# JiehongLin/SAM-6D

Hardware: AMD Instinct MI355X
Metric: RGB-D frames/sec (SAM-6D per-frame hot path: SAM ViT-H encoder + ISM scoring + PEM) (higher is better)
Workload: dtype bf16 (SAM ViT-H: 87 % of the step) + f16 (PEM ViT-B feature extractor) + f32 (ISM scoring, PEM point transformer and pose solvers); 1 GPU; LM-O single object: 32 frames/step/GPU, 640x480 RGB-D -> 1024^2 SAM input, P=128 proposals x 42 templates (scored in groups of 8 frames), 1 instance/frame, 2048 pts (PEM batch 32); sam_frames_per_launch_group=16, pem_vit_dtype=fp16 (set by bench.py; the library default is fp32)

## Files before the change

### include/sam6d_hip.h

```cpp
#ifndef SAM6D_HIP_H
#define SAM6D_HIP_H

#include <stdint.h>

#ifdef __cplusplus
extern "C" {
#endif

#define S6D_OK 0
#define S6D_EINVAL (-1)
#define S6D_ELAUNCH (-2)
#define S6D_EUNSUPPORTED (-3)

#define S6D_ABI_VERSION 136
int s6d_version(void);
int s6d_set_persistent_grid_limit(int max_workgroups);
int s6d_set_gemm_wave_tile(int columns);
int s6d_set_gemm_mfma_shape(int rows);
int s6d_set_gemm_small_tile(int enable);
const char *s6d_strerror(int code);
const char *s6d_last_hip_error(void);


int s6d_fps_f32(const float *xyz, int B, int N, int M, float *tmp, int32_t *idx, void *stream);

int s6d_gather_points_f32(const float *points, const int32_t *idx, int B, int C, int N, int M,
                          float *out, void *stream);

int s6d_ball_query_f32(const float *new_xyz, const float *xyz, int B, int N, int M, float radius,
                       int nsample, int32_t *idx, void *stream);

int s6d_group_points_f32(const float *points, const int32_t *idx, int B, int C, int N, int M, int S,
                         float *out, void *stream);

int s6d_gather_rows_f32(const float *src, const int32_t *idx, int B, int N, int C, int M, float *out,
                        void *stream);

int s6d_segment_seq_sum_f32(const float *x, const int64_t *start, const int64_t *count, int P, int C, float *out,
                            void *stream);

int s6d_pem_sample_indices_f32(const float *keys, long key_stride, const int64_t *count, int P, int n_sample,
                               int64_t *idx, int32_t *overflow, void *stream);

int s6d_pem_mask_boxes_u8(const unsigned char *mask, const float *depth, int P, int H, int W, long min_points,
                          unsigned char *m, int64_t *cnt, unsigned char *ok, int64_t *box, void *stream);

int s6d_pem_compact_cloud_f32(const unsigned char *m, const float *depth, const int64_t *box, const unsigned char *ok, int P,
                              int H, int W, float fx, float fy, float cx, float cy, long cap, int32_t *choose, float *cloud,
                              int64_t *n, void *stream);
int s6d_pem_radius_filter_f32(const float *center, const double *limit, int P, long cap, int32_t *choose, float *cloud,
                              int64_t *n, void *stream);

int s6d_pem_crops_f32(const unsigned char *image, const unsigned char *m, const int64_t *kept, const int64_t *box, int M,
                      int H, int W, int S, int use_mask, const float *mean3_host, const float *std3_host, float *out,
                      void *stream);


int s6d_template_boxes_u8(const unsigned char *mask, int T, int H, int W, int64_t *cnt, int64_t *box, int64_t *tight,
                          void *stream);

int s6d_template_points_f32(const unsigned char *mask, const float *xyz_mm, const int64_t *box, int T, int H, int W, long cap,
                            int32_t *choose, float *pts, int64_t *n, void *stream);

int s6d_template_pem_crops_f32(const unsigned char *images, const unsigned char *mask, const int64_t *box, int T, int H, int W,
                               int S, int use_mask, const float *mean3_host, const float *std3_host, float *out, void *stream);

int s6d_template_ism_crops_f32(const unsigned char *images, const unsigned char *mask, const void *params, int T, int H, int W,
                               int S, int normalize, const float *mean3_host, const float *std3_host, float *out_rgb,
                               float *out_mask, void *stream);


int s6d_raster_views_f32(const float *vertices, const int32_t *faces, const unsigned char *colors, const float *poses, int V, int F,
                         int T, int H, int W, float fx, float fy, float cx, float cy, float znear, float ambient, float diffuse,
                         void *workspace, unsigned char *rgb, unsigned char *mask, float *xyz, float *depth, int32_t *face,
                         int32_t *skipped, void *stream);
long s6d_raster_workspace_bytes(int T, int F, int H, int W);

int s6d_texture_pyramid_u8(const unsigned char *image, int Ht, int Wt, void *pyramid, void *stream);
long s6d_texture_pyramid_bytes(int Ht, int Wt);

int s6d_raster_views_tex_f32(const float *vertices, const int32_t *faces, const float *uv, const void *pyramid, const float *poses,
                             int V, int F, int T, int H, int W, int Ht, int Wt, float fx, float fy, float cx, float cy, float znear,
                             float ambient, float diffuse, void *workspace, unsigned char *rgb, unsigned char *mask, float *xyz,
                             float *depth, int32_t *face, int32_t *level, int32_t *skipped, void *stream);

int s6d_raster_depth_f32(const float *vertices, const int32_t *faces, const float *poses, const float *cams, int V, int F, int T,
                         int H, int W, float znear, void *workspace, float *depth, int32_t *skipped, void *stream);
long s6d_raster_depth_workspace_bytes(int T, int F, int H, int W);


int s6d_pose_err_mssd_mspd_f32(const float *vertices, const float *est, const float *gts, const float *cams, int V, int N, int S,
                               float *mssd, float *mspd, void *stream);

int s6d_vsd_counts_f32(const float *depth_est, const float *depth_gt, const float *depth_test, const int32_t *test_index,
                       const float *cams, const float *scale, int N, int M, int H, int W, float delta, const float *taus_host,
                       int NT, int32_t *uni, int32_t *inter, int32_t *ge, void *stream);

int s6d_gt_visibility_f32(const float *canvas, const float *depth_test, const int32_t *test_index, const float *cams, int N, int M,
                          int H, int W, int mx, int my, float delta, uint8_t *mask, uint8_t *mask_visib, int32_t *counts,
                          int32_t *extents, void *stream);

int s6d_model_diameter_f32(const float *vertices, int V, float *diameter, void *stream);
// ... 282 lines not shown
```

### sam6d_amd/csrc/s6d_attn_common.h

```cpp
#pragma once
#include "s6d_bf16.h"

#ifndef S6D_ATTN_F16
#define S6D_ATTN_F16 0
#endif
#if S6D_ATTN_F16
#define S6D_ATTN_NS s6d_h
#define S6D_ATTN_MFMA16(a, b, c) __builtin_amdgcn_mfma_f32_16x16x32_f16(a, b, c, 0, 0, 0)
#define S6D_ATTN_ONE 0x3C00
#else
#define S6D_ATTN_NS s6d
#define S6D_ATTN_MFMA16(a, b, c) __builtin_amdgcn_mfma_f32_16x16x32_bf16(a, b, c, 0, 0, 0)
#define S6D_ATTN_ONE 0x3F80
#endif

namespace S6D_ATTN_NS {
using namespace s6d;

#if S6D_ATTN_F16
typedef f16x8 bf16x8;
__device__ __forceinline__ u16 f2bf(float f) {
  union { _Float16 b; u16 u; } x;
  x.b = (_Float16)f;
  return x.u;
// ... 149 lines not shown
  union PB { bf16x8 v; u16 h[8]; };
  PB pb[NS][2];
  union VA { bf16x8 v; s16x4 q[2]; };
  if (PRIO) __builtin_amdgcn_s_setprio(0);
  if (kAbl & 4) {
#pragma unroll
    for (int n = 0; n < NS; ++n)
#pragma unroll
      for (int sub = 0; sub < 4; ++sub)
#pragma unroll
        for (int r = 0; r < 4; ++r) pb[n][sub >> 1].h[(sub & 1) * 4 + r] = f2bf(s[n][sub][r]);
  } else {
    constexpr float kDefer = 6.0f;
    float mx[NS];
    bool grow[NS], any_grow = false;
#pragma unroll
    for (int n = 0; n < NS; ++n) {
      float v = s[n][0][0];
#pragma unroll
      for (int sub = 0; sub < SUBS; ++sub)
#pragma unroll
        for (int r = 0; r < 4; ++r) v = fmaxf(v, s[n][sub][r]);
      v = fmaxf(v, __shfl_xor(v, 16));
      v = fmaxf(v, __shfl_xor(v, 32));
      if (MODE == 1) v += thv[n];
      mx[n] = v;
      grow[n] = __any(v - st.m_run[n] > kDefer);
      any_grow |= grow[n];
    }
    S6D_TICK(tk, 3);
    if (any_grow) {
#pragma unroll
      for (int n = 0; n < NS; ++n)
        if (grow[n]) {
          const float m_new = fmaxf(st.m_run[n], mx[n]);
          const float alpha = fast_exp2(st.m_run[n] - m_new);
          st.lacc[n] *= alpha;
#pragma unroll
          for (int dt = 0; dt < C::DT; ++dt) st.oacc[n][dt] *= alpha;
          st.m_run[n] = m_new;
        }
    }
#pragma unroll
    for (int n = 0; n < NS; ++n) {
      const float m_sub = (MODE == 1) ? st.m_run[n] - thv[n] : st.m_run[n];
#pragma unroll
      for (int sub = 0; sub < 4; ++sub)
#pragma unroll
        for (int r = 0; r < 4; ++r)
          pb[n][sub >> 1].h[(sub & 1) * 4 + r] = sub < SUBS ? f2bf(fast_exp2(s[n][sub][r] - m_sub)) : (u16)0;
    }
  }
  if (kAbl & 8) {
#pragma unroll
    for (int n = 0; n < NS; ++n) st.lacc[n][0] += (float)pb[n][0].h[0] + (float)pb[n][1].h[7];
    return;
  }
  union { bf16x8 v; u16 h[8]; } ones;
#pragma unroll
  for (int i = 0; i < 8; ++i) ones.h[i] = S6D_ATTN_ONE;
  S6D_TICK(tk, 4);
  if (PRIO) __builtin_amdgcn_s_setprio(1);
#pragma unroll
  for (int j = 0; j < (SUBS + 1) / 2; ++j) {
    const u16 *vrow = Vl + (32 * j + g * 4 + (c >> 2)) * C::VROW + (c & 3) * 4;
#pragma unroll
    for (int n = 0; n < NS; ++n) st.lacc[n] = S6D_ATTN_MFMA16(ones.v, pb[n][j].v, st.lacc[n]);
#pragma unroll
    for (int dt = 0; dt < C::DT; ++dt) {
      VA va;
      va.q[0] = __builtin_amdgcn_ds_read_tr16_b64_v4i16((S6D_LDS(s16x4) *)(vrow + dt * 16));
      va.q[1] = __builtin_amdgcn_ds_read_tr16_b64_v4i16((S6D_LDS(s16x4) *)(vrow + 16 * C::VROW + dt * 16));
#pragma unroll
      for (int n = 0; n < NS; ++n)
        st.oacc[n][dt] = S6D_ATTN_MFMA16(va.v, pb[n][j].v, st.oacc[n][dt]);
    }
  }
  if (PRIO) __builtin_amdgcn_s_setprio(0);
}

constexpr float kNoMaxSumLimit = 1.2676506e30f;
constexpr float kNoMaxFinite = 3.0e38f;

template <int HD, int NS, bool KSWZ>
__device__ __forceinline__ void process_tile_nomax(const AttnParams &p, const u16 *Kl, const u16 *Vl, StripState<HD, NS> &st,
                                                   const f32x4 (&cbias)[NS][4], const float (&nb)[NS], int lane) {
  using C = Cfg<HD>;
  const int g = lane >> 4, c = lane & 15;
  const int gk = KSWZ ? (g ^ kswz(c)) : g;
  union PB { bf16x8 v; u16 h[8]; };
  PB pb[NS][2];
#pragma unroll
  for (int sub = 0; sub < 4; ++sub) {
    f32x4 acc[NS];
#pragma unroll
    for (int n = 0; n < NS; ++n) acc[n] = cbias[n][sub];
#pragma unroll
    for (int ks = 0; ks < C::KS; ++ks) {
      const bf16x8 a = *reinterpret_cast<const bf16x8 *>(Kl + (sub * 16 + c) * C::KROW + ks * 32 + gk * 8);
#pragma unroll
      for (int n = 0; n < NS; ++n) acc[n] = S6D_ATTN_MFMA16(a, st.qf[n][ks], acc[n]);
    }
#pragma unroll
    for (int n = 0; n < NS; ++n)
#pragma unroll
      for (int r = 0; r < 4; ++r)
        pb[n][sub >> 1].h[(sub & 1) * 4 + r] = f2bf(fast_exp2(__builtin_fmaf(acc[n][r], p.scale_log2, nb[n])));
  }
  union { bf16x8 v; u16 h[8]; } ones;
#pragma unroll
  for (int i = 0; i < 8; ++i) ones.h[i] = S6D_ATTN_ONE;
  union VA { bf16x8 v; s16x4 q[2]; };
#pragma unroll
  for (int j = 0; j < 2; ++j) {
    const u16 *vrow = Vl + (32 * j + g * 4 + (c >> 2)) * C::VROW + (c & 3) * 4;
#pragma unroll
    for (int n = 0; n < NS; ++n) st.lacc[n] = S6D_ATTN_MFMA16(ones.v, pb[n][j].v, st.lacc[n]);
#pragma unroll
    for (int dt = 0; dt < C::DT; ++dt) {
      VA va;
      va.q[0] = __builtin_amdgcn_ds_read_tr16_b64_v4i16((S6D_LDS(s16x4) *)(vrow + dt * 16));
      va.q[1] = __builtin_amdgcn_ds_read_tr16_b64_v4i16((S6D_LDS(s16x4) *)(vrow + 16 * C::VROW + dt * 16));
#pragma unroll
      for (int n = 0; n < NS; ++n) st.oacc[n][dt] = S6D_ATTN_MFMA16(va.v, pb[n][j].v, st.oacc[n][dt]);
    }
  }
}

template <int HD, int THREADS>
struct Stager {
  using C = Cfg<HD>;
  static constexpr int NK = (64 * C::KPARTS + THREADS - 1) / THREADS;
  static constexpr int NV = (64 * C::VPARTS + THREADS - 1) / THREADS;
  uint4 k[NK], v[NV];

  __device__ __forceinline__ void load(const AttnParams &p, int b, int wy, int wx, int head, int key0, int tid) {
#pragma unroll
    for (int n = 0; n < NK; ++n) {
      const int i = min(tid + n * THREADS, 64 * C::KPARTS - 1);
      const int key = i / C::KPARTS, part = i - key * C::KPARTS;
      size_t tok;
      const bool valid = token_offset(p, b, wy, wx, key0 + key, tok);
      k[n] = load_chunk<HD>(p, 1, head, valid, tok, part * 8);
    }
#pragma unroll
    for (int n = 0; n < NV; ++n) {
      const int i = min(tid + n * THREADS, 64 * C::VPARTS - 1);
      const int key = i / C::VPARTS, part = i - key * C::VPARTS;
      size_t tok;
      const bool valid = token_offset(p, b, wy, wx, key0 + key, tok);
      v[n] = load_chunk<HD>(p, 2, head, valid, tok, part * 8);
    }
  }
  __device__ __forceinline__ void store(u16 *Kl, u16 *Vl, int tid, int klim = 64, int vlim = 64) const {
#pragma unroll
    for (int n = 0; n < NK; ++n) {
      const int i = tid + n * THREADS;
      const int key = i / C::KPARTS, part = i - key * C::KPARTS;
      if (i < 64 * C::KPARTS && key < klim) *reinterpret_cast<uint4 *>(Kl + key * C::KROW + part * 8) = k[n];
    }
#pragma unroll
    for (int n = 0; n < NV; ++n) {
      const int i = tid + n * THREADS;
      const int key = i / C::VPARTS, part = i - key * C::VPARTS;
      if (i < 64 * C::VPARTS && key < vlim) *reinterpret_cast<uint4 *>(Vl + key * C::VROW + part * 8) = v[n];
    }
  }
};

template <int HD, int THREADS>
struct StagerLinear {
  using C = Cfg<HD>;
  static constexpr int NK = (64 * C::KPARTS + THREADS - 1) / THREADS;
  static constexpr int NV = (64 * C::VPARTS + THREADS - 1) / THREADS;
  uint4 k[NK], v[NV];
  const u16 *kp[NK], *vp[NV];
  int ko[NK], vo[NV];
  bool kz[NK];
  static_assert(Cfg<HD>::KROW - Cfg<HD>::HDP == 8, "K rows end in a 16-byte pad");

  __device__ __forceinline__ void init(const AttnParams &p, int b, int head, int tid) {
#pragma unroll
    for (int n = 0; n < NK; ++n) {
      const int i = tid + n * THREADS, ic = min(i, 64 * C::KPARTS - 1);
      const int key = ic / C::KPARTS, part = ic - key * C::KPARTS;
      kz[n] = part * 8 >= HD;
      kp[n] = qkv_at(p, (size_t)b * p.T + key, 1, head) + (kz[n] ? HD - 8 : part * 8);
      ko[n] = i < 64 * C::KPARTS ? key * C::KROW + (part ^ kswz(key)) * 8 : (tid & 63) * C::KROW + C::HDP;
    }
#pragma unroll
    for (int n = 0; n < NV; ++n) {
      const int i = tid + n * THREADS, ic = min(i, 64 * C::VPARTS - 1);
      const int key = ic / C::VPARTS, part = ic - key * C::VPARTS;
      vp[n] = qkv_at(p, (size_t)b * p.T + key, 2, head) + part * 8;
      vo[n] = i < 64 * C::VPARTS ? 64 * C::KROW + key * C::VROW + part * 8 : (tid & 63) * C::KROW + C::HDP;
    }
  }
  __device__ __forceinline__ void load(size_t tile_stride_elems, int t) {
#pragma unroll
    for (int n = 0; n < NK; ++n) k[n] = *reinterpret_cast<const uint4 *>(kp[n] + tile_stride_elems * t);
#pragma unroll
    for (int n = 0; n < NV; ++n) v[n] = *reinterpret_cast<const uint4 *>(vp[n] + tile_stride_elems * t);
  }
  __device__ __forceinline__ void store(u16 *Kl) const {
#pragma unroll
    for (int n = 0; n < NK; ++n) *reinterpret_cast<uint4 *>(Kl + ko[n]) = kz[n] ? make_uint4(0, 0, 0, 0) : k[n];
#pragma unroll
    for (int n = 0; n < NV; ++n) *reinterpret_cast<uint4 *>(Kl + vo[n]) = v[n];
  }
// ... 90 lines not shown
```

### sam6d_amd/csrc/s6d_attn_global.h

```cpp
#pragma once
#include "s6d_attn_common.h"

namespace S6D_ATTN_NS {

constexpr bool kGlbPrio = true;

template <int HD, int WAVES, int MODE>
__global__ __launch_bounds__(WAVES * 64) void attn_global_kernel(AttnParams p) {
  using C = Cfg<HD>;
  constexpr int NS = 2;
  static_assert(MODE == 0 || MODE == 2, "attn_global_kernel: table bias (0) or no bias (2); the 64 x 64 grid is attn_global64_kernel's");
  S6D_DYN_LDS(smem);
  constexpr int KBYTES = 64 * C::KROW * 2, VBYTES = 64 * C::VROW * 2;
  auto Kbuf = [&](int r) { return reinterpret_cast<u16 *>(smem + r * (KBYTES + VBYTES)); };
  auto Vbuf = [&](int r) { return reinterpret_cast<u16 *>(smem + r * (KBYTES + VBYTES) + KBYTES); };
  float *tabs = reinterpret_cast<float *>(smem + 2 * (KBYTES + VBYTES));
  const int tid = threadIdx.x, wave = tid >> 6, lane = tid & 63;
  const int c = lane & 15;

  const int nqt = (p.T + WAVES * 16 * NS - 1) / (WAVES * 16 * NS);
  int id = blockIdx.x;
  const int nbh = p.B * p.nh;
  int qt, bh;
  if ((nbh & 7) == 0) {
    const int xcd = id & 7, loc = id >> 3;
    qt = loc % nqt;
    bh = (loc / nqt) * 8 + xcd;
  } else {
    qt = id % nqt;
    bh = id / nqt;
  }
  const int head = bh % p.nh, b = bh / p.nh;
  StripState<HD, NS> st;
  int q0[NS];
#pragma unroll
  for (int n = 0; n < NS; ++n) {
    q0[n] = ((qt * WAVES + wave) * NS + n) * 16;
    load_q<HD>(p, b, 0, 0, head, q0[n], st.qf[n], lane);
    const int qi = min(q0[n] + c, p.T - 1);
    st.qy[n] = div_S(p, qi);
    st.qx[n] = qi - st.qy[n] * p.S;
    st.m_run[n] = -1e30f;
    st.lacc[n] = f32x4{0.f, 0.f, 0.f, 0.f};
#pragma unroll
    for (int i = 0; i < 16; ++i) st.twr[n][i] = 0.f;
#pragma unroll
    for (int dt = 0; dt < C::DT; ++dt) st.oacc[n][dt] = f32x4{0.f, 0.f, 0.f, 0.f};
    st.th[n] = nullptr;
    st.tw[n] = nullptr;
  }
  if (MODE == 0) {
#pragma unroll
    for (int n = 0; n < NS; ++n) {
      float *th = tabs + (size_t)(wave * NS + n) * 2 * 16 * p.LT, *tw = th + 16 * p.LT;
      for (int jt = 0; jt < p.LT / 16; ++jt) {
        build_table<HD, 1>(p.rel_h, jt * 16, 1, st.qf[n], th + jt * 16, p.LT, lane);
        build_table<HD, 1>(p.rel_w, jt * 16, 1, st.qf[n], tw + jt * 16, p.LT, lane);
      }
      st.th[n] = th;
      st.tw[n] = tw;
    }
  }
  const int ntile = p.T / 64;
  StagerLinear<HD, WAVES * 64> sg;
  sg.init(p, b, head, tid);
  const size_t tstride = (size_t)64 * (size_t)p.tok_stride;
  sg.load(tstride, 0);
  __syncthreads();
  sg.store(Kbuf(0));
  __syncthreads();
  auto tile = [&](int t) {
    const float thv[NS] = {0.f, 0.f};
    if (!(kAbl & 2)) process_tile<HD, MODE, NS, true, kGlbPrio>(p, Kbuf(t & 1), Vbuf(t & 1), t * 64, st, thv, lane);
  };
  for (int t = 0; t + 1 < ntile; ++t) {
    if (!(kAbl & 1)) sg.load(tstride, t + 1);
    tile(t);
    if (!(kAbl & 32)) sg.store(Kbuf((t & 1) ^ 1));
    __syncthreads();
  }
  tile(ntile - 1);
#pragma unroll
  for (int n = 0; n < NS; ++n) store_strip<HD>(p, b, 0, 0, head, q0[n], st.lacc[n][0], st.oacc[n], lane);
}

constexpr int G64_THLD = 65;
#ifndef S6D_G64_SLOTS
#define S6D_G64_SLOTS 3
#endif
#ifndef S6D_G64_WAVES
#define S6D_G64_WAVES 8
#endif
#ifndef S6D_G64_NOMAX
#define S6D_G64_NOMAX 1
#endif

template <int HD, int WAVES_, int SLOTS_>
struct G64 {
  using C = Cfg<HD>;
  static constexpr int WAVES = WAVES_, NS = 2, SLOTS = SLOTS_;
  static constexpr int KCH = C::KROW / 8, VCH = C::VROW / 8;
  static constexpr int NPIECE = KCH + VCH;
  static constexpr int PW = (NPIECE + WAVES - 1) / WAVES;
  static constexpr int SLOT = NPIECE * 1024;
  static constexpr int RING = SLOTS * SLOT;
  static constexpr int TABS = WAVES * NS * 16 * G64_THLD * 4;
  static constexpr int LDS = RING + TABS + 16;
  static_assert(NPIECE > WAVES * (PW - 1) && PW >= 2, "every wave has a real piece to repeat");
  static_assert(RING >= WAVES * 16 * 80 * 4, "the prologue's per-wave scratch aliases the ring");
  static_assert(PW * (SLOTS - 2) <= 15 || SLOTS == 2, "vmcnt immediates used below");
};

template <int PW>
__device__ __forceinline__ void g64_wait_tiles(int n) {
  switch (PW * n) {
#define S6D_G64_CASE(k) case k: S6D_VMCNT(k); break;
    S6D_G64_CASE(0) S6D_G64_CASE(3) S6D_G64_CASE(5) S6D_G64_CASE(6) S6D_G64_CASE(9) S6D_G64_CASE(10) S6D_G64_CASE(12)
#undef S6D_G64_CASE
    default: S6D_VMCNT(15); break;
  }
}

template <int HD, int WAVES, int SLOTS>
__global__ __launch_bounds__(WAVES * 64) void attn_global64_kernel(AttnParams p) {
  using C = Cfg<HD>;
  using G = G64<HD, WAVES, SLOTS>;
  constexpr int NS = G::NS, PW = G::PW;
  S6D_DYN_LDS(smem);
  float *tabs = reinterpret_cast<float *>(smem + G::RING);
  const int tid = threadIdx.x, wave = __builtin_amdgcn_readfirstlane(tid >> 6), lane = tid & 63;
  const int g = lane >> 4, c = lane & 15;
  const int nqt = p.T / (WAVES * 16 * NS);
  const int nbh = p.B * p.nh;
  int id = blockIdx.x, qt, bh;
  if ((nbh & 7) == 0) {
    const int xcd = id & 7, loc = id >> 3;
    qt = loc % nqt;
    bh = (loc / nqt) * 8 + xcd;
  } else {
    qt = id % nqt;
    bh = id / nqt;
  }
  const int head = bh % p.nh, b = bh / p.nh;
  StripState<HD, NS> st;
  int q0[NS];
  float *thm[NS];
#pragma unroll
  for (int n = 0; n < NS; ++n) {
    q0[n] = ((qt * WAVES + wave) * NS + n) * 16;
    load_q<HD>(p, b, 0, 0, head, q0[n], st.qf[n], lane);
    st.qy[n] = q0[n] >> 6;
    st.qx[n] = (q0[n] & 63) + c;
    st.m_run[n] = -1e30f;
    st.lacc[n] = f32x4{0.f, 0.f, 0.f, 0.f};
#pragma unroll
    for (int dt = 0; dt < C::DT; ++dt) st.oacc[n][dt] = f32x4{0.f, 0.f, 0.f, 0.f};
    st.th[n] = nullptr;
    st.tw[n] = nullptr;
    float *th = tabs + (size_t)(wave * NS + n) * 16 * G64_THLD;
    float *Gs = reinterpret_cast<float *>(smem) + (size_t)wave * 16 * 80;
    const int q0y = q0[n] >> 6, q0x = q0[n] & 63;
    build_table<HD, 4>(p.rel_h, q0y + 63, -1, st.qf[n], th, G64_THLD, lane);
    build_table<HD, 5>(p.rel_w, q0x, 1, st.qf[n], Gs, 80, lane);
    S6D_WAVE_RENDEZVOUS();
#pragma unroll
    for (int sub = 0; sub < 4; ++sub)
#pragma unroll
      for (int r = 0; r < 4; ++r) st.twr[n][sub * 4 + r] = Gs[c * 80 + (c + 63 - (sub * 16 + g * 4 + r))];
    S6D_WAVE_RENDEZVOUS();
    thm[n] = th;
  }
  const u16 *src[PW];
  long inc[PW];
  int dsto[PW];
  const long tstride = 64L * p.tok_stride;
#pragma unroll
  for (int i = 0; i < PW; ++i) {
    const int q = wave + WAVES * i < G::NPIECE ? wave + WAVES * i : wave + WAVES * (i - 1);
    const bool isk = q < G::KCH;
    const int piece = isk ? q : q - G::KCH, rowch = isk ? G::KCH : G::VCH;
    const int j = piece * 64 + lane;
    const int row = j / rowch, pp = j - row * rowch;
    const int part = isk ? (pp < C::KPARTS ? pp ^ kswz(row) : C::KPARTS) : pp;
    const bool data = part * 8 < HD;
    src[i] = data ? qkv_at(p, (size_t)b * p.T + row, isk ? 1 : 2, head) + part * 8 : reinterpret_cast<const u16 *>(&g_attn_zero16);
    inc[i] = data ? tstride : 0;
    dsto[i] = q * 1024;
  }
  auto issue = [&](int slot) __attribute__((always_inline)) {
#pragma unroll
    for (int i = 0; i < PW; ++i) {
      S6D_LDS(char) *dst = (S6D_LDS(char) *)smem + slot * G::SLOT + dsto[i];
      lds_dma16_m0(src[i], dst);
      src[i] += inc[i];
    }
  };
  const int ntile = p.T / 64;
  constexpr int D = SLOTS - 1;
  static_assert(D >= 1 && D <= 6, "ring depth");
  f32x4 cbias[NS][4];
  {
    const float inv = 1.0f / p.scale_log2;
#pragma unroll
    for (int n = 0; n < NS; ++n)
#pragma unroll
      for (int sub = 0; sub < 4; ++sub)
#pragma unroll
        for (int r = 0; r < 4; ++r) cbias[n][sub][r] = st.twr[n][sub * 4 + r] * inv;
  }
  int *redo = reinterpret_cast<int *>(smem + G::RING + G::TABS);
  const u16 *src0[PW];
#pragma unroll
  for (int i = 0; i < PW; ++i) src0[i] = src[i];
  long long tk[6] = {0, 0, 0, 0, 0, 0}, tsum[5] = {0, 0, 0, 0, 0};
  int slot = 0;
  auto tile_head = [&](int t, float (&thv)[NS]) __attribute__((always_inline)) -> const u16 * {
    S6D_TICK(tk, 0);
    g64_wait_tiles<PW>(min(D - 1, ntile - 1 - t));
    S6D_LGKM0();
    __builtin_amdgcn_s_barrier();
    S6D_TICK(tk, 1);
    if (t + D < ntile && !(kAbl & 1)) issue(slot >= 1 ? slot - 1 : SLOTS - 1);
#pragma unroll
    for (int n = 0; n < NS; ++n) thv[n] = thm[n][c * G64_THLD + t];
    S6D_TICK(tk, 2);
    const u16 *Kl = reinterpret_cast<const u16 *>(smem + slot * G::SLOT);
    slot = slot == SLOTS - 1 ? 0 : slot + 1;
    return Kl;
  };
  auto prime = [&]() __attribute__((always_inline)) {
    __syncthreads();
    if (tid == 0) *redo = 0;
#pragma unroll
    for (int d = 0; d < D; ++d) issue(d);
    slot = 0;
  };
  bool done = false;
  if (S6D_G64_NOMAX && !S6D_G64_TIMING) {
    prime();
    {
      float thv[NS];
      const u16 *Kl = tile_head(0, thv);
      process_tile<HD, 1, NS, true, kGlbPrio>(p, Kl, Kl + 64 * C::KROW, 0, st, thv, lane, tk);
    }
    for (int t = 1; t < ntile; ++t) {
      float thv[NS], nb[NS];
      const u16 *Kl = tile_head(t, thv);
#pragma unroll
      for (int n = 0; n < NS; ++n) nb[n] = thv[n] - st.m_run[n];
      process_tile_nomax<HD, NS, true>(p, Kl, Kl + 64 * C::KROW, st, cbias, nb, lane);
    }
    bool bad = false;
#pragma unroll
    for (int n = 0; n < NS; ++n) {
      bad |= !(st.lacc[n][0] < kNoMaxSumLimit);
#pragma unroll
      for (int dt = 0; dt < C::DT; ++dt)
#pragma unroll
        for (int r = 0; r < 4; ++r) bad |= !(fabsf(st.oacc[n][dt][r]) < kNoMaxFinite);
    }
    if (__any(bad) && lane == 0) *redo = 1;
    __syncthreads();
    done = *redo == 0;
    if (!done) {
#pragma unroll
      for (int n = 0; n < NS; ++n) {
        st.m_run[n] = -1e30f;
        st.lacc[n] = f32x4{0.f, 0.f, 0.f, 0.f};
#pragma unroll
        for (int dt = 0; dt < C::DT; ++dt) st.oacc[n][dt] = f32x4{0.f, 0.f, 0.f, 0.f};
      }
#pragma unroll
      for (int i = 0; i < PW; ++i) src[i] = src0[i];
    }
  }
  if (!done) {
    prime();
    for (int t = 0; t < ntile; ++t) {
      float thv[NS];
      const u16 *Kl = tile_head(t, thv);
      if (!(kAbl & 2)) process_tile<HD, 1, NS, true, kGlbPrio>(p, Kl, Kl + 64 * C::KROW, t * 64, st, thv, lane, tk);
      S6D_TICK(tk, 5);
      if (S6D_G64_TIMING)
#pragma unroll
        for (int i = 0; i < 5; ++i) tsum[i] += tk[i + 1] - tk[i];
    }
  }
#pragma unroll
  for (int n = 0; n < NS; ++n) store_strip<HD>(p, b, 0, 0, head, q0[n], st.lacc[n][0], st.oacc[n], lane);
  if (S6D_G64_TIMING && blockIdx.x == 8 && lane == 0) {
    long long *dbg = reinterpret_cast<long long *>(p.out + (size_t)p.B * p.T * p.nh * HD);
#pragma unroll
    for (int i = 0; i < 5; ++i) dbg[wave * 5 + i] = tsum[i];
  }
}

template <int HD>
static int launch_global(AttnParams p, hipStream_t st) {
  using C = Cfg<HD>;
  const bool bias = p.rel_h != nullptr;
  if (p.T % 64 != 0) return S6D_EUNSUPPORTED;
  if (bias && p.S == 64) {
    using G = G64<HD, S6D_G64_WAVES, S6D_G64_SLOTS>;
    static_assert(G::LDS <= 160 * 1024, "ring + tables fit the CU's LDS");
    launch_lds(attn_global64_kernel<HD, G::WAVES, G::SLOTS>, (unsigned)(p.B * p.nh * (p.T / (G::WAVES * 32))), G::WAVES * 64, G::LDS, st, p);
    return launch_status();
  }
  constexpr int WAVES = 4, NS = 2;
  const size_t ring = (size_t)2 * 64 * (C::KROW + C::VROW) * 2;
  const int nqt = (p.T + WAVES * 16 * NS - 1) / (WAVES * 16 * NS);
  const unsigned grid = (unsigned)(p.B * p.nh * nqt);
  const size_t lds = bias ? ring + (size_t)WAVES * NS * 2 * 16 * p.LT * 4 : ring;
  if (lds > 160 * 1024) return S6D_EUNSUPPORTED;
  if (bias) {
    launch_lds(attn_global_kernel<HD, WAVES, 0>, grid, WAVES * 64, lds, st, p);
  } else {
    launch_lds(attn_global_kernel<HD, WAVES, 2>, grid, WAVES * 64, lds, st, p);
  }
  return launch_status();
}

}
```

### sam6d_amd/csrc/s6d_capi.hip

```cpp
#include "s6d_common.h"

#include <string.h>

namespace s6d {
static thread_local char g_hip_err[256] = {0};
void set_hip_error(hipError_t e) {
  const char *s = hipGetErrorString(e);
  strncpy(g_hip_err, s ? s : "unknown", sizeof(g_hip_err) - 1);
}
}

namespace s6d {
int g_s6d_persistent_grid_limit = 0;
}
extern "C" int s6d_set_persistent_grid_limit(int max_workgroups) {
  if (max_workgroups < 0) return S6D_EINVAL;
  s6d::g_s6d_persistent_grid_limit = max_workgroups;
  return S6D_OK;
}

namespace s6d {
int g_s6d_gemm_wave_tile = 0;
}
extern "C" int s6d_set_gemm_wave_tile(int columns) {
  if (columns != 0 && columns != 64 && columns != 128) return S6D_EINVAL;
  s6d::g_s6d_gemm_wave_tile = columns;
  return S6D_OK;
}

namespace s6d {
int g_s6d_gemm_mfma_shape = 0;
}
extern "C" int s6d_set_gemm_mfma_shape(int rows) {
  if (rows != 0 && rows != 16 && rows != 32) return S6D_EINVAL;
  s6d::g_s6d_gemm_mfma_shape = rows;
  return S6D_OK;
}

namespace s6d {
int g_s6d_gemm_small_tile = 1;
}
extern "C" int s6d_set_gemm_small_tile(int enable) {
  if (enable < 0 || enable > 2) return S6D_EINVAL;
  s6d::g_s6d_gemm_small_tile = enable;
  return S6D_OK;
}

extern "C" int s6d_version(void) { return S6D_ABI_VERSION; }

extern "C" const char *s6d_last_hip_error(void) { return s6d::g_hip_err; }

extern "C" const char *s6d_strerror(int code) {
  switch (code) {
    case S6D_OK: return "ok";
    case S6D_EINVAL: return "invalid argument (size, null pointer or shape)";
    case S6D_ELAUNCH: return "HIP kernel launch failed";
    case S6D_EUNSUPPORTED: return "shape not supported by this build";
    default: return "unknown sam6d_hip error";
  }
}
```

### sam6d_amd/csrc/s6d_common.h

```cpp
#pragma once
#include <hip/hip_runtime.h>
#include <stdint.h>

#include "../../include/sam6d_hip.h"

#ifdef HIPEMU
#define S6D_WAVE_RENDEZVOUS() hipemu::wave_barrier()
#else
#define S6D_WAVE_RENDEZVOUS() do { } while (0)
#endif

namespace s6d {

constexpr int kWave = 64;

void set_hip_error(hipError_t e);

inline int launch_status() {
  hipError_t e = hipGetLastError();
  if (e != hipSuccess) {
    set_hip_error(e);
    return S6D_ELAUNCH;
  }
  return S6D_OK;
}

inline hipStream_t as_stream(void *s) { return reinterpret_cast<hipStream_t>(s); }
extern int g_s6d_persistent_grid_limit;

__device__ __forceinline__ int lane_id() { return threadIdx.x & 63; }

__device__ __forceinline__ float wave_max(float v) {
#pragma unroll
  for (int o = 32; o > 0; o >>= 1) v = fmaxf(v, __shfl_xor(v, o));
  return v;
}
__device__ __forceinline__ float wave_sum(float v) {
#pragma unroll
  for (int o = 32; o > 0; o >>= 1) v += __shfl_xor(v, o);
  return v;
}
__device__ __forceinline__ unsigned long long wave_max_u64(unsigned long long v) {
#pragma unroll
  for (int o = 32; o > 0; o >>= 1) {
    unsigned lo = __shfl_xor((unsigned)(v & 0xffffffffull), o);
    unsigned hi = __shfl_xor((unsigned)(v >> 32), o);
    unsigned long long w = ((unsigned long long)hi << 32) | lo;
    v = w > v ? w : v;
  }
  return v;
}
__device__ __forceinline__ unsigned long long wave_min_u64(unsigned long long v) {
#pragma unroll
  for (int o = 32; o > 0; o >>= 1) {
    const unsigned lo = __shfl_xor((unsigned)(v & 0xffffffffull), o);
    const unsigned hi = __shfl_xor((unsigned)(v >> 32), o);
    const unsigned long long w = ((unsigned long long)hi << 32) | lo;
    v = w < v ? w : v;
  }
  return v;
}
__device__ __forceinline__ int wave_sum_i32(int v) {
#pragma unroll
  for (int o = 32; o > 0; o >>= 1) v += __shfl_xor(v, o);
  return v;
}

__device__ __forceinline__ float gelu_erf(float x) {
  const float ax = fabsf(x);
  const float z = fminf(ax, 6.0f);
  float p = fmaf(z, -1.833880219e-06f, 6.155846495e-05f);
  p = fmaf(z, p, -9.300006204e-04f);
  p = fmaf(z, p, 8.504784666e-03f);
  p = fmaf(z, p, -5.395101011e-02f);
  p = fmaf(z, p, -4.584769309e-01f);
  p = fmaf(z, p, -1.151244164e+00f);
  p = fmaf(z, p, -9.999961853e-01f);
  return fmaf(-ax, __builtin_amdgcn_exp2f(p), fmaxf(x, 0.f));
}
typedef float f32x2 __attribute__((ext_vector_type(2)));
typedef float f32x4 __attribute__((ext_vector_type(4)));
template <typename V>
__device__ __forceinline__ V gelu_erf_poly(V z) {
  V p = __builtin_elementwise_fma(z, (V)(-1.833880219e-06f), (V)(6.155846495e-05f));
  p = __builtin_elementwise_fma(z, p, (V)(-9.300006204e-04f));
  p = __builtin_elementwise_fma(z, p, (V)(8.504784666e-03f));
  p = __builtin_elementwise_fma(z, p, (V)(-5.395101011e-02f));
  p = __builtin_elementwise_fma(z, p, (V)(-4.584769309e-01f));
  p = __builtin_elementwise_fma(z, p, (V)(-1.151244164e+00f));
  return __builtin_elementwise_fma(z, p, (V)(-9.999961853e-01f));
}
__device__ __forceinline__ void gelu_erf4(float *x) {
  const f32x4 z = {fminf(fabsf(x[0]), 6.0f), fminf(fabsf(x[1]), 6.0f), fminf(fabsf(x[2]), 6.0f), fminf(fabsf(x[3]), 6.0f)};
  const f32x4 p = gelu_erf_poly(z);
#pragma unroll
  for (int i = 0; i < 4; ++i) x[i] = fmaf(-fabsf(x[i]), __builtin_amdgcn_exp2f(p[i]), fmaxf(x[i], 0.f));
}

}
```

### sam6d_amd/ops.py

```python
import ctypes

import torch

from . import _lib
from . import policy


def _stream():
    return torch.cuda.current_stream().cuda_stream


def _ptr(t):
    return None if t is None else t.data_ptr()


def _float3(values):
    return (ctypes.c_float * 3)(*[float(v) for v in values])


def _chk(t, dtype, name, ndim=None):
    if not t.is_cuda:
        raise RuntimeError(f"{name} must be a CUDA tensor")
    if not t.is_contiguous():
        raise RuntimeError(f"{name} must be a contiguous tensor")
# ... 1099 lines not shown
        _call("s6d_seq_attention_" + sfx, _ptr(qkv), B, N, int(num_heads), int(C // num_heads), scale, _ptr(out), _stream())
        return out
    H3, M, hd = qkv.shape
    N = int(seq_len)
    if H3 != 3 * num_heads or M % N:
        raise ValueError(f"head-major qkv must be (3 * num_heads, B * N, hd); got {tuple(qkv.shape)} for {num_heads} heads, N = {N}")
    B = M // N
    out = torch.empty(B, N, num_heads * hd, dtype=qkv.dtype, device=qkv.device)
    _call("s6d_seq_attention_strided_" + sfx, _ptr(qkv), hd, num_heads * M * hd, M * hd, B, N, int(num_heads), hd, scale, _ptr(out),
          _stream())
    return out


def gemm_bf16(a, w, bias=None, gelu=False, out=None, max_blocks=0, col_block=0, residual=None, stats_partial=None):
    if not a.is_cuda or not w.is_cuda:
        raise RuntimeError("a and w must be CUDA tensors")
    if a.dtype not in (torch.bfloat16, torch.float16) or w.dtype != a.dtype:
        raise RuntimeError("a and w must both be bfloat16 (or both float16) tensors")
    f16 = a.dtype == torch.float16
    if f16 and (col_block or residual is not None):
        raise RuntimeError("the float16 GEMM has the plain and the GELU epilogue only")
    K = a.shape[-1]
    N = w.shape[0]
    a2 = a.reshape(-1, K)
    if a2.stride(1) != 1 or a2.stride(0) % 8 or a2.data_ptr() % 16:
        a2 = a2.contiguous()
    if w.dim() != 2 or w.shape[1] != K or w.stride(1) != 1 or w.stride(0) % 8:
        raise RuntimeError("w must be (N, K) with contiguous rows")
    if bias is not None:
        _chk(bias, torch.float32, "bias", 1)
    M = a2.shape[0]
    if col_block:
        if out is not None:
            raise RuntimeError("col_block output is allocated by the call")
        out = torch.empty(N // col_block, M, col_block, dtype=torch.bfloat16, device=a.device)
        _call("s6d_gemm_bf16_cblk", _ptr(a2), a2.stride(0), _ptr(w), w.stride(0), _ptr(bias), _ptr(out), N, M, N, K, 1 if gelu else 0,
              int(col_block), int(max_blocks), _stream())
        return out
    if out is None:
        out = torch.empty(M, N, dtype=a.dtype, device=a.device)
    else:
        _chk(out, a.dtype, "out", 2)
        if tuple(out.shape) != (M, N) or out.stride(1) != 1 or out.stride(0) % 8 or out.data_ptr() % 16:
            raise ValueError(f"out must be ({M}, {N}) bf16 with contiguous, 16-byte aligned rows (stride % 8 == 0); got "
                             f"{tuple(out.shape)} strides {tuple(out.stride())}")
    rows = gemm_one_launch_rows(a2.stride(0))
    if residual is not None:
        if gelu or col_block:
            raise RuntimeError("the residual form takes neither GELU nor column blocks")
        _chk(residual, torch.bfloat16, "residual")
        r2 = residual.reshape(-1, N)
        if r2.shape[0] != M:
            raise ValueError(f"residual has {r2.shape[0]} rows, the product {M}")
        if r2.stride(1) != 1 or r2.stride(0) % 8 or r2.data_ptr() % 16:
            raise ValueError("residual rows must be contiguous and 16-byte aligned")
        if stats_partial is not None:
            _chk(stats_partial, torch.float32, "stats_partial")
            if tuple(stats_partial.shape) != (N // 32, 2, M) or not stats_partial.is_contiguous():
                raise ValueError(f"stats_partial must be a contiguous ({N // 32}, 2, {M}) f32 tensor; got {tuple(stats_partial.shape)}")
            if M > rows:
                raise RuntimeError("row statistics are written for one launch: the row count exceeds one 2-GiB slab")
        for r0 in range(0, M, rows):
            r1 = min(M, r0 + rows)
            _call("s6d_gemm_bf16_res", _ptr(a2[r0:r1]), a2.stride(0), _ptr(w), w.stride(0), _ptr(bias), _ptr(r2[r0:r1]), r2.stride(0),
                  _ptr(stats_partial), _ptr(out[r0:r1]), out.stride(0), r1 - r0, N, K, int(max_blocks), _stream())
        return out.reshape(*a.shape[:-1], N)
    if stats_partial is not None:
        raise RuntimeError("stats_partial comes with the residual form")
    for r0 in range(0, M, rows):
        r1 = min(M, r0 + rows)
        _call("s6d_gemm_f16" if f16 else "s6d_gemm_bf16", _ptr(a2[r0:r1]), a2.stride(0), _ptr(w), w.stride(0), _ptr(bias), _ptr(out[r0:r1]),
              out.stride(0), r1 - r0, N, K, 1 if gelu else 0, int(max_blocks), _stream())
    return out.reshape(*a.shape[:-1], N)


def set_geo_embed_form(form):
    _call("s6d_set_geo_embed_form", int(form))


def set_gemm_small_tile(enable):
    _call("s6d_set_gemm_small_tile", int(enable))


def set_gemm_wave_tile(columns):
    _call("s6d_set_gemm_wave_tile", int(columns))


def set_gemm_mfma_shape(rows):
    _call("s6d_set_gemm_mfma_shape", int(rows))


def gemm_one_launch_rows(row_stride, elem_bytes=2):
    return max(256, ((2 ** 31 - 1) // (elem_bytes * int(row_stride))) // 256 * 256)


def ln_stats_finalize(stats_partial, group_size=32, eps=1e-6):
    _chk(stats_partial, torch.float32, "stats_partial", 3)
    if not stats_partial.is_contiguous() or stats_partial.shape[1] != 2:
        raise ValueError("stats_partial must be a contiguous (groups, 2, M) tensor")
    G, _, M = stats_partial.shape
    out = torch.empty(M, 2, dtype=torch.float32, device=stats_partial.device)
    _call("s6d_ln_stats_finalize", _ptr(stats_partial), G, int(group_size), M, eps, _ptr(out), _stream())
    return out


def row_stats(x, eps=1e-6):
    _chk(x, torch.bfloat16, "x")
    C = x.shape[-1]
    x2 = x.reshape(-1, C)
    if x2.stride(1) != 1 or x2.stride(0) % 8 or x2.data_ptr() % 16:
        x2 = x2.contiguous()
    out = torch.empty(x2.shape[0], 2, dtype=torch.float32, device=x.device)
    _call("s6d_row_stats_bf16", _ptr(x2), x2.stride(0), x2.shape[0], C, eps, _ptr(out), _stream())
    return out


def gemm_bf16_lnfold(a, stats, w_folded, col_sums, bias, gelu=False, col_block=0, max_blocks=0):
    _chk(a, torch.bfloat16, "a")
    _chk(w_folded, torch.bfloat16, "w_folded", 2)
    _chk(stats, torch.float32, "stats", 2)
    _chk(col_sums, torch.float32, "col_sums", 1)
    _chk(bias, torch.float32, "bias", 1)
    K, N = a.shape[-1], w_folded.shape[0]
    a2 = a.reshape(-1, K)
    if a2.stride(1) != 1 or a2.stride(0) % 8 or a2.data_ptr() % 16:
        a2 = a2.contiguous()
    M = a2.shape[0]
    if w_folded.shape[1] != K or w_folded.stride(1) != 1 or w_folded.stride(0) % 8:
        raise RuntimeError("w_folded must be (N, K) with contiguous rows")
    if tuple(stats.shape) != (M, 2) or not stats.is_contiguous() or col_sums.numel() != N or bias.numel() != N:
        raise ValueError(f"stats must be ({M}, 2), col_sums and bias ({N},)")
    if M > gemm_one_launch_rows(a2.stride(0)):
        raise RuntimeError("one launch: the row count exceeds one 2-GiB slab")
    if col_block:
        out = torch.empty(N // col_block, M, col_block, dtype=torch.bfloat16, device=a.device)
    else:
        out = torch.empty(M, N, dtype=torch.bfloat16, device=a.device)
    _call("s6d_gemm_bf16_lnfold", _ptr(a2), a2.stride(0), _ptr(stats), _ptr(w_folded), w_folded.stride(0), _ptr(col_sums), _ptr(bias),
          _ptr(out), N, M, N, K, 1 if gelu else 0, int(col_block), int(max_blocks), _stream())
    return out if col_block else out.reshape(*a.shape[:-1], N)


def gemm_fp8(a8, a_scale, w8, w_scale, bias=None, gelu=False, max_blocks=0):
    for t, nm in ((a8, "a8"), (a_scale, "a_scale"), (w8, "w8"), (w_scale, "w_scale")):
        _chk(t, torch.uint8, nm)
    K, N = a8.shape[-1], w8.shape[0]
    a2 = a8.reshape(-1, K)
    M = a2.shape[0]
    if w8.shape != (N, K) or a_scale.numel() != M or w_scale.numel() != N:
        raise ValueError(f"shapes: a8 {tuple(a8.shape)}, a_scale {tuple(a_scale.shape)}, w8 {tuple(w8.shape)}, w_scale {tuple(w_scale.shape)}")
    if bias is not None:
        _chk(bias, torch.float32, "bias", 1)
    out = torch.empty(M, N, dtype=torch.bfloat16, device=a8.device)
    rows = max(256, ((2 ** 31 - 1) // K) // 256 * 256)
    for r0 in range(0, M, rows):
        r1 = min(M, r0 + rows)
        _call("s6d_gemm_fp8", _ptr(a2[r0:r1]), K, _ptr(a_scale.reshape(-1)[r0:r1]), _ptr(w8), K, _ptr(w_scale), _ptr(bias),
              _ptr(out[r0:r1]), N, r1 - r0, N, K, 1 if gelu else 0, int(max_blocks), _stream())
    return out.reshape(*a8.shape[:-1], N)


def gemm_fp8_gelu_mx(a8, a_scale, w8, w_scale, bias=None, max_blocks=0):
    for t, nm in ((a8, "a8"), (a_scale, "a_scale"), (w8, "w8"), (w_scale, "w_scale")):
        _chk(t, torch.uint8, nm)
    K, N = a8.shape[-1], w8.shape[0]
    a2 = a8.reshape(-1, K)
# ... 422 lines not shown
```

Baseline: 168.8 frames/s.

## Software-pipeline global attention: overlap next tile's QK scores with previous PV

Splits the no-max attention tile into a score/softmax stage and a PV stage, then, in half of the waves of the 64x64 global-attention kernel, runs them software-pipelined so tile t's QK^T and exp overlap tile t-1's PV MFMAs. The staggering is meant to desynchronise waves so MFMA and exp/LDS work from different waves interleave better. An extra lifetime slot is added to the K/V LDS ring so a tile's V stays valid one iteration longer, and the rel-w table is rebuilt on the fallback path. It costs more LDS and registers (pb held across iterations), and a runtime knob with default on controls it.

```diff
diff --git a/include/sam6d_hip.h b/include/sam6d_hip.h
--- a/include/sam6d_hip.h
+++ b/include/sam6d_hip.h
@@ -12,12 +12,13 @@
 #define S6D_ELAUNCH (-2)
 #define S6D_EUNSUPPORTED (-3)
 
-#define S6D_ABI_VERSION 136
+#define S6D_ABI_VERSION 137
 int s6d_version(void);
 int s6d_set_persistent_grid_limit(int max_workgroups);
 int s6d_set_gemm_wave_tile(int columns);
 int s6d_set_gemm_mfma_shape(int rows);
 int s6d_set_gemm_small_tile(int enable);
+int s6d_set_global_attn_stagger(int on);
 const char *s6d_strerror(int code);
 const char *s6d_last_hip_error(void);
 
diff --git a/sam6d_amd/csrc/s6d_attn_common.h b/sam6d_amd/csrc/s6d_attn_common.h
--- a/sam6d_amd/csrc/s6d_attn_common.h
+++ b/sam6d_amd/csrc/s6d_attn_common.h
@@ -255,14 +255,14 @@
 constexpr float kNoMaxSumLimit = 1.2676506e30f;
 constexpr float kNoMaxFinite = 3.0e38f;
 
+union TileP { bf16x8 v; u16 h[8]; };
+
 template <int HD, int NS, bool KSWZ>
-__device__ __forceinline__ void process_tile_nomax(const AttnParams &p, const u16 *Kl, const u16 *Vl, StripState<HD, NS> &st,
-                                                   const f32x4 (&cbias)[NS][4], const float (&nb)[NS], int lane) {
+__device__ __forceinline__ void tile_scores_to_p(const AttnParams &p, const u16 *Kl, const StripState<HD, NS> &st,
+                                                 const f32x4 (&cbias)[NS][4], const float (&nb)[NS], int lane, TileP (&pb)[NS][2]) {
   using C = Cfg<HD>;
   const int g = lane >> 4, c = lane & 15;
   const int gk = KSWZ ? (g ^ kswz(c)) : g;
-  union PB { bf16x8 v; u16 h[8]; };
-  PB pb[NS][2];
 #pragma unroll
   for (int sub = 0; sub < 4; ++sub) {
     f32x4 acc[NS];
@@ -280,6 +280,12 @@
       for (int r = 0; r < 4; ++r)
         pb[n][sub >> 1].h[(sub & 1) * 4 + r] = f2bf(fast_exp2(__builtin_fmaf(acc[n][r], p.scale_log2, nb[n])));
   }
+}
+
+template <int HD, int NS>
+__device__ __forceinline__ void tile_pv(const TileP (&pb)[NS][2], const u16 *Vl, StripState<HD, NS> &st, int lane) {
+  using C = Cfg<HD>;
+  const int g = lane >> 4, c = lane & 15;
   union { bf16x8 v; u16 h[8]; } ones;
 #pragma unroll
   for (int i = 0; i < 8; ++i) ones.h[i] = S6D_ATTN_ONE;
@@ -298,6 +304,14 @@
       for (int n = 0; n < NS; ++n) st.oacc[n][dt] = S6D_ATTN_MFMA16(va.v, pb[n][j].v, st.oacc[n][dt]);
     }
   }
+}
+
+template <int HD, int NS, bool KSWZ>
+__device__ __forceinline__ void process_tile_nomax(const AttnParams &p, const u16 *Kl, const u16 *Vl, StripState<HD, NS> &st,
+                                                   const f32x4 (&cbias)[NS][4], const float (&nb)[NS], int lane) {
+  TileP pb[NS][2];
+  tile_scores_to_p<HD, NS, KSWZ>(p, Kl, st, cbias, nb, lane, pb);
+  tile_pv<HD, NS>(pb, Vl, st, lane);
 }
 
 template <int HD, int THREADS>
diff --git a/sam6d_amd/csrc/s6d_attn_global.h b/sam6d_amd/csrc/s6d_attn_global.h
--- a/sam6d_amd/csrc/s6d_attn_global.h
+++ b/sam6d_amd/csrc/s6d_attn_global.h
@@ -85,11 +85,15 @@
 }
 
 constexpr int G64_THLD = 65;
+constexpr int kG64StaggerDefault = 1;
 #ifndef S6D_G64_SLOTS
 #define S6D_G64_SLOTS 3
 #endif
 #ifndef S6D_G64_WAVES
 #define S6D_G64_WAVES 8
+#endif
+#ifndef S6D_G64_STAGGER_ALL
+#define S6D_G64_STAGGER_ALL 0
 #endif
 #ifndef S6D_G64_NOMAX
 #define S6D_G64_NOMAX 1
@@ -103,12 +107,14 @@
   static constexpr int NPIECE = KCH + VCH;
   static constexpr int PW = (NPIECE + WAVES - 1) / WAVES;
   static constexpr int SLOT = NPIECE * 1024;
-  static constexpr int RING = SLOTS * SLOT;
+  static constexpr int LIFE = 1, NSLOT = SLOTS + LIFE;
+  static constexpr int RING = NSLOT * SLOT;
   static constexpr int TABS = WAVES * NS * 16 * G64_THLD * 4;
   static constexpr int LDS = RING + TABS + 16;
   static_assert(NPIECE > WAVES * (PW - 1) && PW >= 2, "every wave has a real piece to repeat");
   static_assert(RING >= WAVES * 16 * 80 * 4, "the prologue's per-wave scratch aliases the ring");
-  static_assert(PW * (SLOTS - 2) <= 15 || SLOTS == 2, "vmcnt immediates used below");
+  static_assert(PW * (SLOTS - 2) <= 15 || SLOTS == 2, "vmcnt immediates used below (the waits count look-ahead tiles: the lifetime slot adds none)");
+  static_assert(LDS <= 160 * 1024, "ring + tables fit the CU's LDS");
 };
 
 template <int PW>
@@ -122,10 +128,10 @@
 }
 
 template <int HD, int WAVES, int SLOTS>
-__global__ __launch_bounds__(WAVES * 64) void attn_global64_kernel(AttnParams p) {
+__global__ __launch_bounds__(WAVES * 64) void attn_global64_kernel(AttnParams p, int stagger) {
   using C = Cfg<HD>;
   using G = G64<HD, WAVES, SLOTS>;
-  constexpr int NS = G::NS, PW = G::PW;
+  constexpr int NS = G::NS, PW = G::PW, NSLOT = G::NSLOT;
   S6D_DYN_LDS(smem);
   float *tabs = reinterpret_cast<float *>(smem + G::RING);
   const int tid = threadIdx.x, wave = __builtin_amdgcn_readfirstlane(tid >> 6), lane = tid & 63;
@@ -145,6 +151,17 @@
   StripState<HD, NS> st;
   int q0[NS];
   float *thm[NS];
+  auto build_twr = [&](int n, int lane) __attribute__((always_inline)) {
+    const int g = lane >> 4, c = lane & 15;
+    float *Gs = reinterpret_cast<float *>(smem) + (size_t)wave * 16 * 80;
+    build_table<HD, 5>(p.rel_w, q0[n] & 63, 1, st.qf[n], Gs, 80, lane);
+    S6D_WAVE_RENDEZVOUS();
+#pragma unroll
+    for (int sub = 0; sub < 4; ++sub)
+#pragma unroll
+      for (int r = 0; r < 4; ++r) st.twr[n][sub * 4 + r] = Gs[c * 80 + (c + 63 - (sub * 16 + g * 4 + r))];
+    S6D_WAVE_RENDEZVOUS();
+  };
 #pragma unroll
   for (int n = 0; n < NS; ++n) {
     q0[n] = ((qt * WAVES + wave) * NS + n) * 16;
@@ -158,16 +175,8 @@
     st.th[n] = nullptr;
     st.tw[n] = nullptr;
     float *th = tabs + (size_t)(wave * NS + n) * 16 * G64_THLD;
-    float *Gs = reinterpret_cast<float *>(smem) + (size_t)wave * 16 * 80;
-    const int q0y = q0[n] >> 6, q0x = q0[n] & 63;
-    build_table<HD, 4>(p.rel_h, q0y + 63, -1, st.qf[n], th, G64_THLD, lane);
-    build_table<HD, 5>(p.rel_w, q0x, 1, st.qf[n], Gs, 80, lane);
-    S6D_WAVE_RENDEZVOUS();
-#pragma unroll
-    for (int sub = 0; sub < 4; ++sub)
-#pragma unroll
-      for (int r = 0; r < 4; ++r) st.twr[n][sub * 4 + r] = Gs[c * 80 + (c + 63 - (sub * 16 + g * 4 + r))];
-    S6D_WAVE_RENDEZVOUS();
+    build_table<HD, 4>(p.rel_h, (q0[n] >> 6) + 63, -1, st.qf[n], th, G64_THLD, lane);
+    build_twr(n, lane);
     thm[n] = th;
   }
   const u16 *src[PW];
@@ -220,12 +229,12 @@
     S6D_LGKM0();
     __builtin_amdgcn_s_barrier();
     S6D_TICK(tk, 1);
-    if (t + D < ntile && !(kAbl & 1)) issue(slot >= 1 ? slot - 1 : SLOTS - 1);
+    if (t + D < ntile && !(kAbl & 1)) issue(slot + D >= NSLOT ? slot + D - NSLOT : slot + D);
 #pragma unroll
     for (int n = 0; n < NS; ++n) thv[n] = thm[n][c * G64_THLD + t];
     S6D_TICK(tk, 2);
     const u16 *Kl = reinterpret_cast<const u16 *>(smem + slot * G::SLOT);
-    slot = slot == SLOTS - 1 ? 0 : slot + 1;
+    slot = slot == NSLOT - 1 ? 0 : slot + 1;
     return Kl;
   };
   auto prime = [&]() __attribute__((always_inline)) {
@@ -243,12 +252,31 @@
       const u16 *Kl = tile_head(0, thv);
       process_tile<HD, 1, NS, true, kGlbPrio>(p, Kl, Kl + 64 * C::KROW, 0, st, thv, lane, tk);
     }
-    for (int t = 1; t < ntile; ++t) {
+    if (!(stagger && (S6D_G64_STAGGER_ALL || wave >= WAVES / 2))) {
+      for (int t = 1; t < ntile; ++t) {
+        float thv[NS], nb[NS];
+        const u16 *Kl = tile_head(t, thv);
+#pragma unroll
+        for (int n = 0; n < NS; ++n) nb[n] = thv[n] - st.m_run[n];
+        process_tile_nomax<HD, NS, true>(p, Kl, Kl + 64 * C::KROW, st, cbias, nb, lane);
+      }
+    } else if (ntile > 1) {
+      TileP pb[NS][2];
       float thv[NS], nb[NS];
-      const u16 *Kl = tile_head(t, thv);
+      const u16 *Kl = tile_head(1, thv);
 #pragma unroll
       for (int n = 0; n < NS; ++n) nb[n] = thv[n] - st.m_run[n];
-      process_tile_nomax<HD, NS, true>(p, Kl, Kl + 64 * C::KROW, st, cbias, nb, lane);
+      tile_scores_to_p<HD, NS, true>(p, Kl, st, cbias, nb, lane, pb);
+      const u16 *Vl = Kl + 64 * C::KROW;
+      for (int t = 2; t < ntile; ++t) {
+        Kl = tile_head(t, thv);
+        tile_pv<HD, NS>(pb, Vl, st, lane);
+#pragma unroll
+        for (int n = 0; n < NS; ++n) nb[n] = thv[n] - st.m_run[n];
+        tile_scores_to_p<HD, NS, true>(p, Kl, st, cbias, nb, lane, pb);
+        Vl = Kl + 64 * C::KROW;
+      }
+      tile_pv<HD, NS>(pb, Vl, st, lane);
     }
     bool bad = false;
 #pragma unroll
@@ -272,6 +300,10 @@
       }
 #pragma unroll
       for (int i = 0; i < PW; ++i) src[i] = src0[i];
+      int lane_again = lane;
+      S6D_PIN(lane_again);
+#pragma unroll
+      for (int n = 0; n < NS; ++n) build_twr(n, lane_again);
     }
   }
   if (!done) {
@@ -302,8 +334,8 @@
   if (p.T % 64 != 0) return S6D_EUNSUPPORTED;
   if (bias && p.S == 64) {
     using G = G64<HD, S6D_G64_WAVES, S6D_G64_SLOTS>;
-    static_assert(G::LDS <= 160 * 1024, "ring + tables fit the CU's LDS");
-    launch_lds(attn_global64_kernel<HD, G::WAVES, G::SLOTS>, (unsigned)(p.B * p.nh * (p.T / (G::WAVES * 32))), G::WAVES * 64, G::LDS, st, p);
+    launch_lds(attn_global64_kernel<HD, G::WAVES, G::SLOTS>, (unsigned)(p.B * p.nh * (p.T / (G::WAVES * 32))), G::WAVES * 64, G::LDS, st, p,
+               g_s6d_global_attn_stagger < 0 ? kG64StaggerDefault : g_s6d_global_attn_stagger);
     return launch_status();
   }
   constexpr int WAVES = 4, NS = 2;
diff --git a/sam6d_amd/csrc/s6d_capi.hip b/sam6d_amd/csrc/s6d_capi.hip
--- a/sam6d_amd/csrc/s6d_capi.hip
+++ b/sam6d_amd/csrc/s6d_capi.hip
@@ -46,6 +46,15 @@
   return S6D_OK;
 }
 
+namespace s6d {
+int g_s6d_global_attn_stagger = -1;
+}
+extern "C" int s6d_set_global_attn_stagger(int on) {
+  if (on < -1 || on > 1) return S6D_EINVAL;
+  s6d::g_s6d_global_attn_stagger = on;
+  return S6D_OK;
+}
+
 extern "C" int s6d_version(void) { return S6D_ABI_VERSION; }
 
 extern "C" const char *s6d_last_hip_error(void) { return s6d::g_hip_err; }
diff --git a/sam6d_amd/csrc/s6d_common.h b/sam6d_amd/csrc/s6d_common.h
--- a/sam6d_amd/csrc/s6d_common.h
+++ b/sam6d_amd/csrc/s6d_common.h
@@ -27,6 +27,7 @@
 
 inline hipStream_t as_stream(void *s) { return reinterpret_cast<hipStream_t>(s); }
 extern int g_s6d_persistent_grid_limit;
+extern int g_s6d_global_attn_stagger;
 
 __device__ __forceinline__ int lane_id() { return threadIdx.x & 63; }
 
diff --git a/sam6d_amd/ops.py b/sam6d_amd/ops.py
--- a/sam6d_amd/ops.py
+++ b/sam6d_amd/ops.py
@@ -1205,6 +1205,10 @@
     _call("s6d_set_gemm_small_tile", int(enable))
 
 
+def set_global_attn_stagger(on):
+    _call("s6d_set_global_attn_stagger", -1 if on is None else int(on))
+
+
 def set_gemm_wave_tile(columns):
     _call("s6d_set_gemm_wave_tile", int(columns))
 
```

Result: no change. 169.6 frames/s (median of 6 runs) (+0.5%).
